# avi2924/Speech-Intent-Recognizer

Hardware: AMD Instinct MI355X
Metric: utterances/sec (16 kHz, 3 s clips), inference: HIP STFT+mel+CNN/BiGRU forward + argmax (higher is better)
Workload: dtype f32

## Files before the change

speech-intent-recognizer_amd/csrc/model_infer.hip:

```cpp
#include "bf16x6_kernels.h"
#include "f16x3_kernels.h"
#include "conv_wino_bf16x6_kernel.h"
#include "conv_wino2_bf16x6_kernel.h"
#include "gru_frag_prep.h"

namespace {

enum WsBuf {
    WS_A1 = 0,
    WS_A2,
    WS_X0,
    WS_GI,
    WS_Y0,
    WS_Y1,
    WS_CTX,
    WS_PAD,
    WS_XZ,
    WS_BN,
    WS_WHT,
    WS_XS,
    WS_WS,
    WS_WCB,
    WS_GXB,
    WS_GFL,
    WS_COUNT
};

struct Dims {
    int B, T, wp1, wp2, wp3, S;
    int tw2, tw3, k2max, k3max;
};

bool make_dims(int batch, int t_frames, Dims* d) {
    d->B = batch; d->T = t_frames;
    d->wp1 = t_frames / 2; d->wp2 = d->wp1 / 2; d->wp3 = d->wp2 / 2; d->S = d->wp3;
    d->tw2 = (d->wp1 + 1) / 2; d->tw3 = (d->wp2 + 1) / 2; d->k2max = (d->tw2 + 3) / 4; d->k3max = (d->tw3 + 3) / 4;
    return batch > 0 && d->S >= 1 && d->S <= ATT_MAX_S && batch <= 65535;
}

struct PadTabs { size_t e0, d1, d3, tab2, tab3, rows, count; };
PadTabs pad_tabs(const Dims& d) {
    PadTabs t;
    const size_t n = (size_t)d.B + 1;
    t.e0 = 0; t.d1 = d.B; t.d3 = t.d1 + n; t.tab2 = t.d3 + n; t.tab3 = t.tab2 + 1 + n * d.k2max; t.rows = t.tab3 + 1 + n * d.k3max;
    t.count = t.rows + 1 + n * d.S;
    return t;
}

void ws_sizes(const Dims& d, size_t* bytes) {
    const size_t B = d.B + 1;
    bytes[WS_A1] = B * 32 * d.wp1 * 32 * 4;
    bytes[WS_A2] = B * 16 * d.wp2 * 64 * 4;
    bytes[WS_X0] = B * d.S * 1024 * 4;
    bytes[WS_GI] = B * d.S * 1536 * 4;
    bytes[WS_Y0] = (size_t)d.B * d.S * 512 * 4;
    bytes[WS_Y1] = (size_t)d.B * d.S * 512 * 4;
    bytes[WS_CTX] = (size_t)d.B * 512 * 4;
    bytes[WS_PAD] = pad_tabs(d).count * 4;
    bytes[WS_XZ] = (size_t)64 * d.T * 4;
    bytes[WS_BN] = (size_t)2 * 224 * 4;
    bytes[WS_WHT] = 4 * GRU_FRAG_BYTES;
    bytes[WS_XS] = B * d.S * 1024 * 2 * 2;
    bytes[WS_WS] = ((size_t)2 * 2 * 768 * 1024 + (size_t)2 * 2 * 768 * 512) * 2;
    bytes[WS_WCB] = ((size_t)3 * 32 * 16 * 64 + (size_t)3 * 64 * 16 * 128 + (size_t)3 * 64 * 9 * 128) * 2;
    bytes[WS_GXB] = 0;
    bytes[WS_GFL] = 0;
}

size_t ws_layout(const Dims& d, size_t* off) {
    size_t bytes[WS_COUNT], pos = 0;
    ws_sizes(d, bytes);
    for (int i = 0; i < WS_COUNT; ++i) {
        off[i] = pos;
        pos += sir_align_up(bytes[i], 256);
    }
    return pos;
}

static __global__ __launch_bounds__(256) void pad_extent_kernel(const float* __restrict__ x, int T, int* __restrict__ e0) {
    const unsigned* xb = reinterpret_cast<const unsigned*>(x) + (size_t)blockIdx.x * 64 * T;
    int last = -1;
    for (int c = threadIdx.x; c < T; c += 256) {
        unsigned acc = 0;
#pragma unroll 32
        for (int r = 0; r < 64; ++r) acc |= xb[(size_t)r * T + c];
        if (acc) last = c;
    }
#pragma unroll
    for (int o = 32; o > 0; o >>= 1) last = max(last, __shfl_xor(last, o));
    __shared__ int wl[4];
    if ((threadIdx.x & 63) == 0) wl[threadIdx.x >> 6] = last;
    __syncthreads();
    if (threadIdx.x == 0) e0[blockIdx.x] = max(max(wl[0], wl[1]), max(wl[2], wl[3])) + 1;
}

static __global__ __launch_bounds__(1024) void pad_tables_kernel(const int* __restrict__ e0, Dims d, int* __restrict__ d1o, int* __restrict__ d3o,
                                                                 int* __restrict__ tab2, int* __restrict__ tab3, int* __restrict__ prow,
                                                                 float* __restrict__ xz) {
    const int tid = threadIdx.x;
    for (int i = tid; i < 64 * d.T; i += 1024) xz[i] = 0.0f;
    const int nu = d.B + 1, per = (nu + 1023) / 1024, u0 = min(nu, tid * per), u1 = min(nu, u0 + per);
    auto need = [&](int u, int& c1, int& c3, int& k2, int& k3) {
        if (u == d.B) { c1 = d.wp1; c3 = d.S; k2 = d.k2max; k3 = d.k3max; return; }
        c3 = min(d.S, (e0[u] + 14) / 8);
        const int c2 = min(d.wp2, 2 * c3 + 1);
        c1 = min(d.wp1, 2 * c2 + 1);
        k2 = (c2 + 3) / 4; k3 = (c3 + 3) / 4;
    };
    int s2 = 0, s3 = 0, sr = 0, c1, c3, k2, k3;
    for (int u = u0; u < u1; ++u) { need(u, c1, c3, k2, k3); s2 += k2; s3 += k3; sr += c3; }
    __shared__ int p2[1024], p3[1024], pr[1024];
    p2[tid] = s2; p3[tid] = s3; pr[tid] = sr;
    __syncthreads();
    for (int o = 1; o < 1024; o <<= 1) {
        const int a2 = tid >= o ? p2[tid - o] : 0, a3 = tid >= o ? p3[tid - o] : 0, ar = tid >= o ? pr[tid - o] : 0;
        __syncthreads();
        p2[tid] += a2; p3[tid] += a3; pr[tid] += ar;
        __syncthreads();
    }
    int o2 = p2[tid] - s2, o3 = p3[tid] - s3, orw = pr[tid] - sr;
    for (int u = u0; u < u1; ++u) {
        need(u, c1, c3, k2, k3);
        d1o[u] = c1; d3o[u] = c3;
        for (int k = 0; k < k2; ++k) tab2[1 + o2 + k] = u * d.tw2 + 4 * k;
        for (int k = 0; k < k3; ++k) tab3[1 + o3 + k] = u * d.tw3 + 4 * k;
        for (int s = 0; s < c3; ++s) prow[1 + orw + s] = u * d.S + s;
        o2 += k2; o3 += k3; orw += c3;
    }
    if (tid == 1023) { tab2[0] = p2[1023]; tab3[0] = p3[1023]; prow[0] = pr[1023]; }
}

}

extern "C" size_t sir_model_workspace_bytes(const sir_handle* h, int batch, int t_frames, int train) {
    (void)h;
    if (train) return sir_train_workspace_bytes_impl(batch, t_frames);
    Dims d;
    if (!make_dims(batch, t_frames, &d)) return 0;
    size_t off[WS_COUNT];
    return ws_layout(d, off);
}

extern "C" int sir_model_workspace_offsets(const sir_handle* h, int batch, int t_frames, int train, size_t* offsets,
                                           int n) {
    (void)h; (void)train;
    Dims d;
    if (!make_dims(batch, t_frames, &d) || !offsets) { sir_set_error("sir_model_workspace_offsets: bad shape"); return SIR_EINVAL; }
    size_t off[WS_COUNT];
    ws_layout(d, off);
    for (int i = 0; i < n && i < WS_COUNT; ++i) offsets[i] = off[i];
    return WS_COUNT;
}

#define SIR_KCHECK() SIR_HIP_TRY(hipGetLastError())

extern "C" int sir_model_infer(sir_handle* h, const sir_model_weights* w, const float* feats, int batch, int t_frames,
                               float* logits, int64_t* argmax, void* workspace, size_t workspace_bytes, void* stream_) {
    if (!h || !w || !feats || !logits || !workspace) { sir_set_error("sir_model_infer: NULL argument"); return SIR_EINVAL; }
    Dims d;
    if (!make_dims(batch, t_frames, &d)) {
        sir_set_error("sir_model_infer: unsupported shape batch=%d t_frames=%d (need t_frames >= 8)", batch, t_frames);
        return SIR_EINVAL;
    }
    if (h->cfg.n_mels != 64) { sir_set_error("sir_model_infer: the model is wired for 64 mels (models.py:23)"); return SIR_EUNSUPPORTED; }
    if (w->num_classes < 1 || w->num_classes > 64) { sir_set_error("sir_model_infer: num_classes=%d", w->num_classes); return SIR_EINVAL; }
    size_t off[WS_COUNT];
    const size_t need = ws_layout(d, off);
    if (workspace_bytes < need) { sir_set_error("sir_model_infer: workspace %zu < %zu", workspace_bytes, need); return SIR_ENOMEM; }
    if (((uintptr_t)workspace & 255) != 0) { sir_set_error("sir_model_infer: workspace must be 256-byte aligned"); return SIR_EINVAL; }
    hipStream_t st = (hipStream_t)stream_;
    char* ws = (char*)workspace;
    float* a1 = (float*)(ws + off[WS_A1]);
    float* a2 = (float*)(ws + off[WS_A2]);
    float* x0 = (float*)(ws + off[WS_X0]);
    float* gi = (float*)(ws + off[WS_GI]);
    float* y0 = (float*)(ws + off[WS_Y0]);
    float* y1 = (float*)(ws + off[WS_Y1]);
    float* ctx = (float*)(ws + off[WS_CTX]);
    float* bns = (float*)(ws + off[WS_BN]);
    float* bnt = bns + 224;
    float* wht = (float*)(ws + off[WS_WHT]);
    unsigned short* xs = (unsigned short*)(ws + off[WS_XS]);
    unsigned short* wsl0 = (unsigned short*)(ws + off[WS_WS]);
    unsigned short* wsl1 = wsl0 + (size_t)2 * 2 * 768 * 1024;
    unsigned short* wcb2 = (unsigned short*)(ws + off[WS_WCB]);
    unsigned short* wcb3 = wcb2 + (size_t)3 * 32 * 16 * 64;
    unsigned short* wcb3d = wcb3 + (size_t)3 * 64 * 16 * 128;
    const int B = d.B, S = d.S;
    const PadTabs pt = pad_tabs(d);
    int* const ptab = (int*)(ws + off[WS_PAD]);
    float* const xz = (float*)(ws + off[WS_XZ]);

    Wino2Geo geo2, geo3;
    const bool w2 = sir_conv_stage_fits(2, wino2_geo(B + 1, 32, d.wp1, 64, &geo2)) && sir_conv_stage_fits(3, wino2_geo(B + 1, 16, d.wp2, 128, &geo3));
    const int BT = w2 ? B + 1 : B;

    const long long prep_key = ((long long)B << 32) | (unsigned)d.T;
    sir_handle::PrepEntry* pe = nullptr;
    for (auto& e : h->prep)
        if (e.ws == workspace) pe = &e;
    const bool reuse_prep = pe && h->weights_version != 0 && pe->version == h->weights_version && pe->key == prep_key;
    if (!reuse_prep) {
        SirProfScope prof(h, SIR_K_PREP, st);
        const int bn_c[3] = {32, 64, 128}, bn_o[3] = {0, 32, 96};
        for (int i = 0; i < 3; ++i)
            hipLaunchKernelGGL(prep_bn_kernel, dim3(1), dim3(128), 0, st, w->bn_w[i], w->bn_b[i], w->bn_mean[i], w->bn_var[i],
                               bns + bn_o[i], bnt + bn_o[i], bn_c[i]);
        for (int i = 0; i < 4; ++i) sir_prep_whh_quad(st, w->gru_w_hh[i], (unsigned char*)wht + (size_t)i * GRU_FRAG_BYTES);
        if (w2) hipLaunchKernelGGL(prep_conv_w_wino_f16x3_kernel, dim3((32 * 16 * 64 + 255) / 256), dim3(256), 0, st, w->conv_w[1], wcb2, 32, 64, h->status);
        else hipLaunchKernelGGL(prep_conv_w_wino_bf16x3_kernel, dim3((32 * 16 * 64 + 255) / 256), dim3(256), 0, st, w->conv_w[1], wcb2, 32, 64);
        if (w2) hipLaunchKernelGGL(prep_conv_w_wino_f16x3_kernel, dim3((64 * 16 * 128 + 255) / 256), dim3(256), 0, st, w->conv_w[2], wcb3, 64, 128, h->status);
        else hipLaunchKernelGGL(prep_conv_w_wino_bf16x3_kernel, dim3((64 * 16 * 128 + 255) / 256), dim3(256), 0, st, w->conv_w[2], wcb3, 64, 128);
        hipLaunchKernelGGL(prep_conv_w_bf16x3_kernel, dim3((64 * 9 * 128 + 255) / 256), dim3(256), 0, st, w->conv_w[2], wcb3d, 64, 128);
        for (int dir = 0; dir < 2; ++dir) {
            hipLaunchKernelGGL(split2h_kernel, dim3(384), dim3(256), 0, st, w->gru_w_ih[dir], 1024, wsl0 + (size_t)dir * 2 * 768 * 1024, (size_t)768, 1024);
            hipLaunchKernelGGL(split2h_kernel, dim3(192), dim3(256), 0, st, w->gru_w_ih[2 + dir], 512, wsl1 + (size_t)dir * 2 * 768 * 512, (size_t)768, 512);
        }
        if (!pe) { pe = &h->prep[h->prep_next]; h->prep_next = (h->prep_next + 1) % 4; }
        pe->ws = workspace; pe->version = h->weights_version; pe->key = prep_key;
    }
    SIR_KCHECK();

    {
        SirProfScope prof(h, SIR_K_CONV1, st);
        if (w2) {
            hipLaunchKernelGGL(pad_extent_kernel, dim3(B), dim3(256), 0, st, feats, d.T, ptab + pt.e0);
            hipLaunchKernelGGL(pad_tables_kernel, dim3(1), dim3(1024), 0, st, (const int*)(ptab + pt.e0), d, ptab + pt.d1, ptab + pt.d3,
                               ptab + pt.tab2, ptab + pt.tab3, ptab + pt.rows, xz);
        }
        hipLaunchKernelGGL(conv1_mfma_bn_relu_pool_kernel, dim3((d.wp1 + C1_PCOLS - 1) / C1_PCOLS, 1, BT), dim3(256), 0, st, feats,
                           w->conv_w[0], bns, bnt, a1, 64, d.T, 32, d.wp1, (const float*)xz, B, w2 ? (const int*)(ptab + pt.d1) : (const int*)nullptr);
    }
    {
        SirProfScope prof(h, SIR_K_CONV2, st);
        if (w2)
            SIR_HIP_TRY((launch_conv_wino2<32, 64, 0>(st, &h->attr_wino2[0], a1, (const unsigned short*)wcb2, bns + 32, bnt + 32, a2, BT, 32, d.wp1,
                                                    (float2*)nullptr, h->zero_page, h->num_cus, ptab + pt.tab2, (B + 1) * d.k2max)));
        else
            hipLaunchKernelGGL((conv3x3_wino_bf16x6_kernel<32, 64, 0>), dim3(((d.wp1 + 1) / 2 + 1) / 2, 1, B), dim3(256), WINO_LDS_BYTES, st,
                               a1, (const unsigned short*)wcb2, bns + 32, bnt + 32, a2, 32, d.wp1, 16, d.wp2, (float2*)nullptr);
    }
    {
        SirProfScope prof(h, SIR_K_CONV3, st);
        if (w2)
            SIR_HIP_TRY((launch_conv_wino2<64, 128, 1>(st, &h->attr_wino2[1], a2, (const unsigned short*)wcb3, bns + 96, bnt + 96, x0, BT, 16, d.wp2,
                                                     (float2*)xs, h->zero_page, h->num_cus, ptab + pt.tab3, (B + 1) * d.k3max)));
        else
            hipLaunchKernelGGL((conv3x3_bf16x6_ns_kernel<64, 128, 2, 2, 1, 0, 2, 1, 1>), dim3((d.wp2 + 7) / 8, 1, B), dim3(256), conv_ns_lds_bytes(2, 2, 2), st,
                               a2, (const unsigned short*)wcb3d, bns + 96, bnt + 96, x0, 16, d.wp2, 8, d.wp3, (float2*)xs);
    }
    SIR_KCHECK();

    const int M = B * S;
    {
        SirProfScope prof(h, SIR_K_GEMM_IH0, st);
        if (w2)
            SIR_HIP_TRY(launch_gemm_nt_f16x3_gather(h, st, (const unsigned short*)xs, (const unsigned short*)wsl0,
                                                    (const unsigned short*)(wsl0 + (size_t)2 * 768 * 1024), w->gru_b_ih[0], w->gru_b_ih[1], gi, 1536,
                                                    (const int*)(ptab + pt.rows), BT * S, 768, 1024));
        else
            SIR_HIP_TRY(launch_gemm_nt_f16x3(h, st, (const unsigned short*)xs, (const unsigned short*)wsl0,
                                             (const unsigned short*)(wsl0 + (size_t)2 * 768 * 1024), w->gru_b_ih[0], w->gru_b_ih[1], gi, 1536, M, 768, 1024));
    }
    {
        SirProfScope prof(h, SIR_K_GRU0, st);
        if (sir_cluster_enter(h, st) != SIR_OK) return SIR_EHIP;
        const int rc = sir_launch_gru_quad(h, st, false, gi, w->gru_w_hh[0], w->gru_w_hh[1], w->gru_b_hh[0], w->gru_b_hh[1], y0, B, S, nullptr,
                                           xs, wht, (unsigned char*)wht + GRU_FRAG_BYTES, w2 ? (const int*)(ptab + pt.d3) : (const int*)nullptr);
        if (rc != SIR_OK) return rc;
        if (sir_cluster_leave(h, st) != SIR_OK) return SIR_EHIP;
    }
    {
        SirProfScope prof(h, SIR_K_GEMM_IH1, st);
        SIR_HIP_TRY(launch_gemm_nt_f16x3(h, st, (const unsigned short*)xs, (const unsigned short*)wsl1,
                                         (const unsigned short*)(wsl1 + (size_t)2 * 768 * 512), w->gru_b_ih[2], w->gru_b_ih[3], gi, 1536, M, 768, 512));
    }
    {
        SirProfScope prof(h, SIR_K_GRU1, st);
        if (sir_cluster_enter(h, st) != SIR_OK) return SIR_EHIP;
        const int rc = sir_launch_gru_quad(h, st, false, gi, w->gru_w_hh[2], w->gru_w_hh[3], w->gru_b_hh[2], w->gru_b_hh[3], y1, B, S, nullptr,
                                           nullptr, (unsigned char*)wht + 2 * GRU_FRAG_BYTES, (unsigned char*)wht + 3 * GRU_FRAG_BYTES);
        if (rc != SIR_OK) return rc;
        if (sir_cluster_leave(h, st) != SIR_OK) return SIR_EHIP;
    }
    SIR_KCHECK();

    {
        SirProfScope prof(h, SIR_K_ATTN, st);
        hipLaunchKernelGGL(attention_pool_kernel, dim3(B), dim3(256), 0, st, y1, w->attn_w, w->attn_b, ctx, S, w->fc_w, w->fc_b,
                           w->num_classes, logits, (long long*)argmax);
    }
    SIR_KCHECK();
    return SIR_OK;
}
```

speech-intent-recognizer_amd/csrc/model_kernels.h:

```cpp
#pragma once
#include "sir_internal.h"

typedef float f32x16 __attribute__((ext_vector_type(16)));
typedef float mk_f32x2 __attribute__((ext_vector_type(2)));

#define SIR_BN_EPS 1e-5f


static __global__ void prep_bn_kernel(const float* __restrict__ g, const float* __restrict__ b, const float* __restrict__ mean,
                               const float* __restrict__ var, float* __restrict__ scale, float* __restrict__ shift, int c) {
    const int i = blockIdx.x * blockDim.x + threadIdx.x;
    if (i >= c) return;
    const float s = g[i] / sqrtf(var[i] + SIR_BN_EPS);
    scale[i] = s;
    shift[i] = b[i] - mean[i] * s;
}

constexpr int C1_PROWS = 4, C1_PCOLS = 32;
constexpr int C1_TR = 2 * C1_PROWS + 2, C1_TC = 2 * C1_PCOLS + 2;

static __global__ __launch_bounds__(256, 4) void conv1_mfma_bn_relu_pool_kernel(
    const float* __restrict__ x, const float* __restrict__ w, const float* __restrict__ scale,
    const float* __restrict__ shift, float* __restrict__ out, int H, int W, int Hp, int Wp,
    const float* __restrict__ xtail, int nx, const int* __restrict__ lim) {
    __shared__ float tiles[2][C1_TR * C1_TC];
    const int b = blockIdx.z, px0 = blockIdx.x * C1_PCOLS;
    const int wlim = lim ? min(Wp, lim[b]) : Wp;
    if (px0 >= wlim) return;
    const int tid = threadIdx.x, lane = tid & 63, wv = tid >> 6, j = lane & 31, kh = lane >> 5;
    const float* xb = b < nx ? x + (size_t)b * H * W : xtail;
    constexpr int NPRE = (C1_TR * C1_TC + 255) / 256;
    float pre[NPRE];
    auto fetch = [&](int py0) {
#pragma unroll
        for (int q = 0; q < NPRE; ++q) {
            const int i = tid + 256 * q, ty = i / C1_TC, tx = i - ty * C1_TC;
            const int gy = 2 * py0 - 1 + ty, gx = 2 * px0 - 1 + tx;
            pre[q] = (i < C1_TR * C1_TC && gy >= 0 && gy < H && gx >= 0 && gx < W) ? xb[(size_t)gy * W + gx] : 0.0f;
        }
    };
    fetch(0);
    float wa[5];
    int boff[5];
#pragma unroll
    for (int s = 0; s < 5; ++s) {
        const int tap = 2 * s + kh;
        wa[s] = tap < 9 ? w[j * 9 + tap] : 0.0f;
        const int tc = tap < 9 ? tap : 8;
        boff[s] = (tc / 3) * C1_TC + (tc % 3) + j;
    }
    float sc[16], sh[16];
#pragma unroll
    for (int r = 0; r < 16; ++r) {
        const int ch = (r & 3) + 8 * (r >> 2) + 4 * kh;
        sc[r] = scale[ch]; sh[r] = shift[ch];
    }
    const bool odd = j & 1;
    int it = 0;
    for (int py0 = 0; py0 < Hp; py0 += C1_PROWS, ++it) {
        float* tile = tiles[it & 1];
#pragma unroll
        for (int q = 0; q < NPRE; ++q)
            if (tid + 256 * q < C1_TR * C1_TC) tile[tid + 256 * q] = pre[q];
        __syncthreads();
        if (py0 + C1_PROWS < Hp) fetch(py0 + C1_PROWS);
        const int py = py0 + wv;
        if (py >= Hp) continue;
        const float* trow = tile + (2 * wv) * C1_TC;
#pragma unroll
        for (int h = 0; h < 2; ++h) {
            if (px0 + 16 * h >= wlim) break;
            f32x16 acc0, acc1;
#pragma unroll
            for (int r = 0; r < 16; ++r) { acc0[r] = 0.0f; acc1[r] = 0.0f; }
#pragma unroll
            for (int s = 0; s < 5; ++s) {
                const float b0 = trow[boff[s] + 32 * h], b1 = trow[boff[s] + 32 * h + C1_TC];
                acc0 = __builtin_amdgcn_mfma_f32_32x32x2f32(wa[s], b0, acc0, 0, 0, 0);
                acc1 = __builtin_amdgcn_mfma_f32_32x32x2f32(wa[s], b1, acc1, 0, 0, 0);
            }
            float m[16];
#pragma unroll
            for (int r = 0; r < 16; r += 2) {
                const mk_f32x2 s2 = {sc[r], sc[r + 1]}, h2 = {sh[r], sh[r + 1]};
                const mk_f32x2 y0 = __builtin_elementwise_fma((mk_f32x2){acc0[r], acc0[r + 1]}, s2, h2);
                const mk_f32x2 y1 = __builtin_elementwise_fma((mk_f32x2){acc1[r], acc1[r + 1]}, s2, h2);
                const float v0 = fmaxf(y0.x, y1.x), v1 = fmaxf(y0.y, y1.y);
                const float nb0 = __builtin_bit_cast(float, __builtin_amdgcn_update_dpp(0, __builtin_bit_cast(int, v0), 0xB1, 0xF, 0xF, true));
                const float nb1 = __builtin_bit_cast(float, __builtin_amdgcn_update_dpp(0, __builtin_bit_cast(int, v1), 0xB1, 0xF, 0xF, true));
                m[r] = fmaxf(fmaxf(v0, nb0), 0.0f);
                m[r + 1] = fmaxf(fmaxf(v1, nb1), 0.0f);
            }
            const int px = px0 + 16 * h + (j >> 1);
            const float4 lo = odd ? make_float4(m[8], m[9], m[10], m[11]) : make_float4(m[0], m[1], m[2], m[3]);
            const float4 hi = odd ? make_float4(m[12], m[13], m[14], m[15]) : make_float4(m[4], m[5], m[6], m[7]);
            if (px < wlim) {
                float* o = out + (((size_t)b * Hp + py) * Wp + px) * 32 + 4 * kh + (odd ? 16 : 0);
                *reinterpret_cast<float4*>(o) = lo;
                *reinterpret_cast<float4*>(o + 8) = hi;
            }
        }
    }
}

constexpr int GB_M = 128, GB_N = 64, GB_K = 32, GB_S = GB_K + 4;

constexpr int GRU_H = 256, GRU_BW = 2;
constexpr int GRU_NPART = 4;
constexpr int GRU_KPER4 = 64 / GRU_NPART;
constexpr int GRU_KREG4 = 3;
constexpr int GRU_KLDS4 = 2;
constexpr int GRU_KSTR4 = GRU_KPER4 - GRU_KREG4 - GRU_KLDS4;
constexpr int GRU_NQ = (GRU_BW + GRU_NPART - 1) / GRU_NPART;
constexpr int GRU_THREADS = 256 * GRU_NPART;
constexpr size_t GRU_LDS_BYTES =
    (size_t)(GRU_NPART * GRU_KLDS4 * 3 * 256 * 4 + GRU_BW * GRU_H + GRU_NPART * GRU_BW * 3 * GRU_H) * 4;

__device__ __forceinline__ float sigmoidf_(float x) { return 1.0f / (1.0f + expf(-x)); }

template <int NB>
__device__ __forceinline__ void gru_fma4(float (&acc)[NB], const float4 w, const float4 (&h4)[NB]) {
#pragma unroll
    for (int bb = 0; bb < NB; ++bb) {
        acc[bb] = fmaf(w.x, h4[bb].x, acc[bb]); acc[bb] = fmaf(w.y, h4[bb].y, acc[bb]);
        acc[bb] = fmaf(w.z, h4[bb].z, acc[bb]); acc[bb] = fmaf(w.w, h4[bb].w, acc[bb]);
    }
}

constexpr int ATT_MAX_S = 256;

static __global__ __launch_bounds__(256) void attention_pool_kernel(const float* __restrict__ y, const float* __restrict__ aw,
                                                             const float* __restrict__ ab, float* __restrict__ ctx,
                                                             int S, const float* __restrict__ fcw,
                                                             const float* __restrict__ fcb, int C,
                                                             float* __restrict__ logits, long long* __restrict__ amax) {
    __shared__ float sc[ATT_MAX_S];
    __shared__ float cs[512];
    __shared__ float lg[64];
    const int b = blockIdx.x, tid = threadIdx.x, lane = tid & 63, wv = tid >> 6;
    const float* yb = y + (size_t)b * S * 512;
    float a[8];
#pragma unroll
    for (int i = 0; i < 8; ++i) a[i] = aw[lane + 64 * i];
    for (int t0 = 4 * wv; t0 < S; t0 += 16) {
        float v[4][8];
#pragma unroll
        for (int k = 0; k < 4; ++k)
#pragma unroll
            for (int i = 0; i < 8; ++i) v[k][i] = (t0 + k < S) ? yb[(size_t)(t0 + k) * 512 + lane + 64 * i] : 0.0f;
#pragma unroll
        for (int k = 0; k < 4; ++k) {
            float d = 0.0f;
#pragma unroll
            for (int i = 0; i < 8; ++i) d = fmaf(v[k][i], a[i], d);
#pragma unroll
            for (int o = 32; o > 0; o >>= 1) d += __shfl_xor(d, o);
            if (lane == 0 && t0 + k < S) sc[t0 + k] = d + ab[0];
        }
    }
    __syncthreads();
    __shared__ float ex[ATT_MAX_S];
    float mx = -INFINITY;
    for (int t = 0; t < S; ++t) mx = fmaxf(mx, sc[t]);
    if (tid < S) ex[tid] = expf(sc[tid] - mx);
    __syncthreads();
    float den = 0.0f;
    for (int t = 0; t < S; ++t) den += ex[t];
    __syncthreads();
    if (tid < S) ex[tid] = ex[tid] / den;
    __syncthreads();
    for (int c = tid; c < 512; c += 256) {
        float acc = 0.0f;
        for (int t = 0; t < S; ++t) acc = fmaf(ex[t], yb[(size_t)t * 512 + c], acc);
        ctx[(size_t)b * 512 + c] = acc;
        cs[c] = acc;
    }
    if (!logits) return;
    __syncthreads();
    for (int j = tid >> 3; j < C; j += 32) {
        const int part = tid & 7;
        const float4* wr = reinterpret_cast<const float4*>(fcw + (size_t)j * 512 + part * 64);
        const float4* cr = reinterpret_cast<const float4*>(cs + part * 64);
        float d = 0.0f;
#pragma unroll
        for (int i = 0; i < 16; ++i) {
            const float4 wv4 = wr[i], c4 = cr[i];
            d = fmaf(c4.x, wv4.x, d); d = fmaf(c4.y, wv4.y, d); d = fmaf(c4.z, wv4.z, d); d = fmaf(c4.w, wv4.w, d);
        }
        d += __shfl_xor(d, 1); d += __shfl_xor(d, 2); d += __shfl_xor(d, 4);
        if (part == 0) {
            d += fcb[j];
            lg[j] = d;
            logits[(size_t)b * C + j] = d;
        }
    }
    if (!amax) return;
    __syncthreads();
    if (tid == 0) {
        float best = lg[0];
        int bi = 0;
        for (int c = 1; c < C; ++c)
            if (lg[c] > best) { best = lg[c]; bi = c; }
        amax[b] = bi;
    }
}
```

Baseline: 730,800.

## Fuse pad-extent scan into a per-utterance conv1 kernel with LDS-resident input

Adds a conv1 kernel that loads a whole utterance's 64xT feature map into LDS once, computes the nonzero extent (replacing the separate pad_extent kernel), and runs the MFMA conv+BN+ReLU+pool only up to the needed padded width. It also writes the tail padding row values directly, so pad_tables no longer has to zero the xz buffer. The goal is fewer launches and less redundant global reads and tile reloads. In exchange, the new path only applies for T up to 240 with 16-byte-aligned input, and uses large LDS footprint with 1024-thread blocks, which may limit occupancy.

```diff
diff --git a/speech-intent-recognizer_amd/csrc/model_infer.hip b/speech-intent-recognizer_amd/csrc/model_infer.hip
--- a/speech-intent-recognizer_amd/csrc/model_infer.hip
+++ b/speech-intent-recognizer_amd/csrc/model_infer.hip
@@ -98,14 +98,14 @@
                                                                  int* __restrict__ tab2, int* __restrict__ tab3, int* __restrict__ prow,
                                                                  float* __restrict__ xz) {
     const int tid = threadIdx.x;
-    for (int i = tid; i < 64 * d.T; i += 1024) xz[i] = 0.0f;
+    if (xz)
+        for (int i = tid; i < 64 * d.T; i += 1024) xz[i] = 0.0f;
     const int nu = d.B + 1, per = (nu + 1023) / 1024, u0 = min(nu, tid * per), u1 = min(nu, u0 + per);
     auto need = [&](int u, int& c1, int& c3, int& k2, int& k3) {
         if (u == d.B) { c1 = d.wp1; c3 = d.S; k2 = d.k2max; k3 = d.k3max; return; }
-        c3 = min(d.S, (e0[u] + 14) / 8);
-        const int c2 = min(d.wp2, 2 * c3 + 1);
-        c1 = min(d.wp1, 2 * c2 + 1);
-        k2 = (c2 + 3) / 4; k3 = (c3 + 3) / 4;
+        const PadNeed n = pad_need(e0[u], d.S, d.wp2, d.wp1);
+        c1 = n.c1; c3 = n.c3;
+        k2 = (n.c2 + 3) / 4; k3 = (n.c3 + 3) / 4;
     };
     int s2 = 0, s3 = 0, sr = 0, c1, c3, k2, k3;
     for (int u = u0; u < u1; ++u) { need(u, c1, c3, k2, k3); s2 += k2; s3 += k3; sr += c3; }
@@ -223,13 +223,23 @@
 
     {
         SirProfScope prof(h, SIR_K_CONV1, st);
-        if (w2) {
-            hipLaunchKernelGGL(pad_extent_kernel, dim3(B), dim3(256), 0, st, feats, d.T, ptab + pt.e0);
+        const bool utt = w2 && d.T <= C1U_TMAX && ((uintptr_t)feats & 15) == 0;
+        if (utt) {
+            int R = 1;
+            while (R < C1U_RMAX && B * R < h->num_cus) R *= 2;
+            hipLaunchKernelGGL(conv1_utt_bn_relu_pool_kernel, dim3(B * R), dim3(1024), 0, st, feats, w->conv_w[0], bns, bnt, a1, d.T, S, R, B,
+                               ptab + pt.e0);
             hipLaunchKernelGGL(pad_tables_kernel, dim3(1), dim3(1024), 0, st, (const int*)(ptab + pt.e0), d, ptab + pt.d1, ptab + pt.d3,
-                               ptab + pt.tab2, ptab + pt.tab3, ptab + pt.rows, xz);
+                               ptab + pt.tab2, ptab + pt.tab3, ptab + pt.rows, (float*)nullptr);
+        } else {
+            if (w2) {
+                hipLaunchKernelGGL(pad_extent_kernel, dim3(B), dim3(256), 0, st, feats, d.T, ptab + pt.e0);
+                hipLaunchKernelGGL(pad_tables_kernel, dim3(1), dim3(1024), 0, st, (const int*)(ptab + pt.e0), d, ptab + pt.d1, ptab + pt.d3,
+                                   ptab + pt.tab2, ptab + pt.tab3, ptab + pt.rows, xz);
+            }
+            hipLaunchKernelGGL(conv1_mfma_bn_relu_pool_kernel, dim3((d.wp1 + C1_PCOLS - 1) / C1_PCOLS, 1, BT), dim3(256), 0, st, feats,
+                               w->conv_w[0], bns, bnt, a1, 64, d.T, 32, d.wp1, (const float*)xz, B, w2 ? (const int*)(ptab + pt.d1) : (const int*)nullptr);
         }
-        hipLaunchKernelGGL(conv1_mfma_bn_relu_pool_kernel, dim3((d.wp1 + C1_PCOLS - 1) / C1_PCOLS, 1, BT), dim3(256), 0, st, feats,
-                           w->conv_w[0], bns, bnt, a1, 64, d.T, 32, d.wp1, (const float*)xz, B, w2 ? (const int*)(ptab + pt.d1) : (const int*)nullptr);
     }
     {
         SirProfScope prof(h, SIR_K_CONV2, st);
diff --git a/speech-intent-recognizer_amd/csrc/model_kernels.h b/speech-intent-recognizer_amd/csrc/model_kernels.h
--- a/speech-intent-recognizer_amd/csrc/model_kernels.h
+++ b/speech-intent-recognizer_amd/csrc/model_kernels.h
@@ -18,6 +18,21 @@
 
 constexpr int C1_PROWS = 4, C1_PCOLS = 32;
 constexpr int C1_TR = 2 * C1_PROWS + 2, C1_TC = 2 * C1_PCOLS + 2;
+
+__device__ __forceinline__ void c1_bn_relu_pool(const f32x16& acc0, const f32x16& acc1, const float (&sc)[16], const float (&sh)[16],
+                                                float (&m)[16]) {
+#pragma unroll
+    for (int r = 0; r < 16; r += 2) {
+        const mk_f32x2 s2 = {sc[r], sc[r + 1]}, h2 = {sh[r], sh[r + 1]};
+        const mk_f32x2 y0 = __builtin_elementwise_fma((mk_f32x2){acc0[r], acc0[r + 1]}, s2, h2);
+        const mk_f32x2 y1 = __builtin_elementwise_fma((mk_f32x2){acc1[r], acc1[r + 1]}, s2, h2);
+        const float v0 = fmaxf(y0.x, y1.x), v1 = fmaxf(y0.y, y1.y);
+        const float nb0 = __builtin_bit_cast(float, __builtin_amdgcn_update_dpp(0, __builtin_bit_cast(int, v0), 0xB1, 0xF, 0xF, true));
+        const float nb1 = __builtin_bit_cast(float, __builtin_amdgcn_update_dpp(0, __builtin_bit_cast(int, v1), 0xB1, 0xF, 0xF, true));
+        m[r] = fmaxf(fmaxf(v0, nb0), 0.0f);
+        m[r + 1] = fmaxf(fmaxf(v1, nb1), 0.0f);
+    }
+}
 
 static __global__ __launch_bounds__(256, 4) void conv1_mfma_bn_relu_pool_kernel(
     const float* __restrict__ x, const float* __restrict__ w, const float* __restrict__ scale,
@@ -103,6 +118,131 @@
     }
 }
 
+struct PadNeed { int c1, c2, c3; };
+__device__ __forceinline__ PadNeed pad_need(int e0, int S, int wp2, int wp1) {
+    PadNeed n;
+    n.c3 = min(S, (e0 + 14) / 8);
+    n.c2 = min(wp2, 2 * n.c3 + 1);
+    n.c1 = min(wp1, 2 * n.c2 + 1);
+    return n;
+}
+
+constexpr int C1U_TMAX = 240;
+constexpr int C1U_LW = C1U_TMAX + 2;
+constexpr int C1U_TILE = 66 * C1U_LW + 32;
+constexpr int C1U_RMAX = 8;
+
+static __global__ __launch_bounds__(1024) void conv1_utt_bn_relu_pool_kernel(
+    const float* __restrict__ x, const float* __restrict__ w, const float* __restrict__ scale, const float* __restrict__ shift,
+    float* __restrict__ out, int T, int S, int R, int B, int* __restrict__ e0o) {
+    constexpr int Hp = 32;
+    __shared__ float tile[C1U_TILE];
+    __shared__ int wl[16];
+    __shared__ float tv[32];
+    constexpr int LW = C1U_LW;
+    const int Wp = T / 2;
+    const int b = blockIdx.x / R, rg = blockIdx.x - b * R;
+    const int tid = threadIdx.x, lane = tid & 63, wv = __builtin_amdgcn_readfirstlane(tid >> 6), j = lane & 31, kh = lane >> 5;
+    const float4* xb = reinterpret_cast<const float4*>(x + (size_t)b * 64 * T);
+    const int n4 = 16 * T;
+    float4 pre[4];
+#pragma unroll
+    for (int q = 0; q < 4; ++q) {
+        const int i = tid + 1024 * q;
+        pre[q] = i < n4 ? xb[i] : make_float4(0.0f, 0.0f, 0.0f, 0.0f);
+    }
+    float wa[5];
+    int boff[5];
+#pragma unroll
+    for (int s = 0; s < 5; ++s) {
+        const int tap = 2 * s + kh;
+        wa[s] = tap < 9 ? w[j * 9 + tap] : 0.0f;
+        const int tc = tap < 9 ? tap : 8;
+        boff[s] = (tc / 3) * LW + (tc % 3) + j;
+    }
+    float sc[16], sh[16];
+#pragma unroll
+    for (int r = 0; r < 16; ++r) {
+        const int ch = (r & 3) + 8 * (r >> 2) + 4 * kh;
+        sc[r] = scale[ch]; sh[r] = shift[ch];
+    }
+    const bool odd = j & 1;
+    if (tid < 2 * LW + 160) {
+        int i = tid, o;
+        if (i < 2 * LW) o = i < LW ? i : 65 * LW + i - LW;
+        else if ((i -= 2 * LW) < 128) o = (1 + (i & 63)) * LW + (i < 64 ? 0 : T + 1);
+        else o = 66 * LW + i - 128;
+        tile[o] = 0.0f;
+    }
+    if (wv == 0) {
+        f32x16 z;
+#pragma unroll
+        for (int r = 0; r < 16; ++r) z[r] = 0.0f;
+        float m[16];
+        c1_bn_relu_pool(z, z, sc, sh, m);
+        const float4 lo = odd ? make_float4(m[8], m[9], m[10], m[11]) : make_float4(m[0], m[1], m[2], m[3]);
+        const float4 hi = odd ? make_float4(m[12], m[13], m[14], m[15]) : make_float4(m[4], m[5], m[6], m[7]);
+        if (j < 2) {
+            float* o = tv + 4 * kh + (odd ? 16 : 0);
+            *reinterpret_cast<float4*>(o) = lo;
+            *reinterpret_cast<float4*>(o + 8) = hi;
+        }
+    }
+    int last = -1;
+    int row, col;
+    auto put = [&](float v) {
+        tile[(row + 1) * LW + col + 1] = v;
+        if (__builtin_bit_cast(unsigned, v)) last = max(last, col);
+        if (++col == T) { ++row; col = 0; }
+    };
+#pragma unroll
+    for (int q = 0; q < 4; ++q) {
+        const int i = tid + 1024 * q;
+        if (i < n4) {
+            row = (4 * i) / T; col = 4 * i - row * T;
+            put(pre[q].x); put(pre[q].y); put(pre[q].z); put(pre[q].w);
+        }
+    }
+#pragma unroll
+    for (int o = 32; o > 0; o >>= 1) last = max(last, __shfl_xor(last, o));
+    if (lane == 0) wl[wv] = last;
+    __syncthreads();
+#pragma unroll
+    for (int k = 0; k < 16; ++k) last = max(last, wl[k]);
+    const int e0 = __builtin_amdgcn_readfirstlane(last + 1);
+    if (rg == 0 && tid == 0) e0o[b] = e0;
+    const int d1 = pad_need(e0, S, Wp / 2, Wp).c1;
+    {
+        const int tot = Hp * Wp * 8, per = (tot + (int)gridDim.x - 1) / (int)gridDim.x, i1 = min(tot, ((int)blockIdx.x + 1) * per);
+        float4* ot = reinterpret_cast<float4*>(out + (size_t)B * Hp * Wp * 32);
+        for (int i = (int)blockIdx.x * per + tid; i < i1; i += 1024) ot[i] = reinterpret_cast<const float4*>(tv)[i & 7];
+    }
+    const int nh = (d1 + 15) >> 4, nrow = Hp / R, units = nrow * nh;
+    for (int u = wv; u < units; u += 16) {
+        const int pr = u / nh, hh = u - pr * nh, py = rg * nrow + pr;
+        const float* trow = tile + 2 * py * LW + 32 * hh;
+        f32x16 acc0, acc1;
+#pragma unroll
+        for (int r = 0; r < 16; ++r) { acc0[r] = 0.0f; acc1[r] = 0.0f; }
+#pragma unroll
+        for (int s = 0; s < 5; ++s) {
+            const float b0 = trow[boff[s]], b1 = trow[boff[s] + LW];
+            acc0 = __builtin_amdgcn_mfma_f32_32x32x2f32(wa[s], b0, acc0, 0, 0, 0);
+            acc1 = __builtin_amdgcn_mfma_f32_32x32x2f32(wa[s], b1, acc1, 0, 0, 0);
+        }
+        float m[16];
+        c1_bn_relu_pool(acc0, acc1, sc, sh, m);
+        const int px = 16 * hh + (j >> 1);
+        const float4 lo = odd ? make_float4(m[8], m[9], m[10], m[11]) : make_float4(m[0], m[1], m[2], m[3]);
+        const float4 hi = odd ? make_float4(m[12], m[13], m[14], m[15]) : make_float4(m[4], m[5], m[6], m[7]);
+        if (px < d1) {
+            float* o = out + (((size_t)b * Hp + py) * Wp + px) * 32 + 4 * kh + (odd ? 16 : 0);
+            *reinterpret_cast<float4*>(o) = lo;
+            *reinterpret_cast<float4*>(o + 8) = hi;
+        }
+    }
+}
+
 constexpr int GB_M = 128, GB_N = 64, GB_K = 32, GB_S = GB_K + 4;
 
 constexpr int GRU_H = 256, GRU_BW = 2;
```

New measurement: 747,100 (median of 6 runs). 1.02x the previous value.
